# Fabstir/fabstir-vectordb

Hardware: NVIDIA B200
Metric: QPS @ recall@10>=0.95, 1M x 384 IVF (higher is better)
Workload: dtype f32

## Files before the change

### fabstir_vectordb_b200/csrc/common.cuh

```cuda
#pragma once

#include <cuda_runtime.h>
#include <stdint.h>

#include <string>

namespace fvdb {

constexpr uint64_t KEY_NONE = 0xFFFFFFFFFFFFFFFFull;
constexpr uint32_t ID_NONE = 0xFFFFFFFFu;

__host__ __device__ __forceinline__ uint64_t make_key(float dist, uint32_t id) {
#ifdef __CUDA_ARCH__
    return ((uint64_t)__float_as_uint(dist) << 32) | id;
#else
    union { float f; uint32_t u; } c;
    c.f = dist;
    return ((uint64_t)c.u << 32) | id;
#endif
}
__host__ __device__ __forceinline__ uint32_t key_id(uint64_t k) { return (uint32_t)k; }
__device__ __forceinline__ float key_dist(uint64_t k) { return __uint_as_float((uint32_t)(k >> 32)); }

constexpr int METRIC_L2 = 0, METRIC_COS = 1, METRIC_DOT = 2;
// ... 92 lines not shown
        for (int j = 0; j < 8; ++j) {
            const float4 qq = q4[i + j];
            float t, u;
            t = __fsub_rn(qq.x, x[j].x); u = __fsub_rn(qq.x, y[j].x);
            acc0 = __fadd_rn(acc0, __fmul_rn(t, t)); acc1 = __fadd_rn(acc1, __fmul_rn(u, u));
            t = __fsub_rn(qq.y, x[j].y); u = __fsub_rn(qq.y, y[j].y);
            acc0 = __fadd_rn(acc0, __fmul_rn(t, t)); acc1 = __fadd_rn(acc1, __fmul_rn(u, u));
            t = __fsub_rn(qq.z, x[j].z); u = __fsub_rn(qq.z, y[j].z);
            acc0 = __fadd_rn(acc0, __fmul_rn(t, t)); acc1 = __fadd_rn(acc1, __fmul_rn(u, u));
            t = __fsub_rn(qq.w, x[j].w); u = __fsub_rn(qq.w, y[j].w);
            acc0 = __fadd_rn(acc0, __fmul_rn(t, t)); acc1 = __fadd_rn(acc1, __fmul_rn(u, u));
        }
    }
    for (; i < n4; ++i) {
        const float4 xx = __ldg(a4 + i), yy = __ldg(b4 + i), qq = q4[i];
        float t, u;
        t = __fsub_rn(qq.x, xx.x); u = __fsub_rn(qq.x, yy.x);
        acc0 = __fadd_rn(acc0, __fmul_rn(t, t)); acc1 = __fadd_rn(acc1, __fmul_rn(u, u));
        t = __fsub_rn(qq.y, xx.y); u = __fsub_rn(qq.y, yy.y);
        acc0 = __fadd_rn(acc0, __fmul_rn(t, t)); acc1 = __fadd_rn(acc1, __fmul_rn(u, u));
        t = __fsub_rn(qq.z, xx.z); u = __fsub_rn(qq.z, yy.z);
        acc0 = __fadd_rn(acc0, __fmul_rn(t, t)); acc1 = __fadd_rn(acc1, __fmul_rn(u, u));
        t = __fsub_rn(qq.w, xx.w); u = __fsub_rn(qq.w, yy.w);
        acc0 = __fadd_rn(acc0, __fmul_rn(t, t)); acc1 = __fadd_rn(acc1, __fmul_rn(u, u));
    }
    d0 = __fsqrt_rn(acc0);
    d1 = __fsqrt_rn(acc1);
}
#endif

inline int div_up(int a, int b) { return (a + b - 1) / b; }
inline uint64_t div_up64(uint64_t a, uint64_t b) { return (a + b - 1) / b; }

}
```

### fabstir_vectordb_b200/csrc/exact_scan.cu

```cuda
#include "common.cuh"
#include "kernels.cuh"

namespace fvdb {

namespace {

constexpr int TQ = 32;
constexpr int TR = 128;
constexpr int DK = 32;
constexpr int NT = 256;
constexpr int QS_LD = TQ + 4;
constexpr int XS_LD = TR + 4;

__device__ __forceinline__ void warp_insert(uint64_t* list, int k, uint64_t cand, int lane) {
    int cnt = 0;
    for (int i = lane; i < k; i += 32) cnt += (list[i] <= cand) ? 1 : 0;
#pragma unroll
    for (int o = 16; o > 0; o >>= 1) cnt += __shfl_xor_sync(0xffffffffu, cnt, o);
    const int pos = cnt;
    for (int base = ((k - 1) / 32) * 32; base >= 0 && base + 31 > pos; base -= 32) {
        int i = base + lane;
        uint64_t tmp = 0;
        bool mv = (i > pos) && (i < k);
        if (mv) tmp = list[i - 1];
// ... 233 lines not shown
    const uint32_t qt = i / nsplit, sp = i % nsplit;
    const uint32_t rows = row_end - row_begin;
    const uint32_t tiles = (rows + TR - 1) / TR;
    const uint32_t t0 = (uint32_t)(((uint64_t)tiles * sp) / nsplit);
    const uint32_t t1 = (uint32_t)(((uint64_t)tiles * (sp + 1)) / nsplit);
    ScanItem it;
    it.row_begin = row_begin + t0 * TR;
    it.row_end = min(row_end, row_begin + t1 * TR);
    it.pair_begin = qt * TQ;
    it.pair_count = min((uint32_t)TQ, nq - qt * TQ);
    it.slot = sp;
    it.identity = 1;
    it.sub = 0;
    if (it.row_begin >= it.row_end) it.pair_count = 0;
    items[i] = it;
}

cudaError_t launch_build_identity_items(ScanItem* items, uint32_t nq, uint32_t row_begin,
                                        uint32_t row_end, uint32_t nsplit, uint32_t* n_items_out,
                                        cudaStream_t stream) {
    const uint32_t n_qt = (nq + TQ - 1) / TQ;
    const uint32_t n = n_qt * nsplit;
    *n_items_out = n;
    if (n == 0) return cudaSuccess;
    build_identity_items_kernel<<<(n + 255) / 256, 256, 0, stream>>>(items, nq, row_begin, row_end,
                                                                    nsplit);
    return cudaGetLastError();
}

uint32_t exact_scan_tq() { return TQ; }
uint32_t exact_scan_tr() { return TR; }


constexpr uint32_t NEAREST_BIT = 0x80000000u;
__global__ void probe_hist_kernel(const uint64_t* __restrict__ coarse_keys, uint32_t n_pairs,
                                  uint32_t nprobe, uint32_t* __restrict__ list_cnt) {
    const uint32_t i = blockIdx.x * blockDim.x + threadIdx.x;
    if (i >= n_pairs) return;
    const uint64_t key = coarse_keys[i];
    if (key == KEY_NONE) return;
    atomicAdd(&list_cnt[key_id(key)], 1u);
    if (i % nprobe == 0) atomicOr(&list_cnt[key_id(key)], NEAREST_BIT);
}

__device__ __forceinline__ uint64_t block_excl_scan_u64(uint64_t v, uint64_t* warp_tot, uint64_t* total) {
    const int lane = threadIdx.x & 31, w = threadIdx.x >> 5;
    uint64_t inc = v;
#pragma unroll
    for (int o = 1; o < 32; o <<= 1) {
        const uint64_t n = __shfl_up_sync(0xffffffffu, inc, o);
        if (lane >= o) inc += n;
    }
    if (lane == 31) warp_tot[w] = inc;
    __syncthreads();
    if (w == 0) {
        uint64_t t = warp_tot[lane];
        uint64_t ti = t;
#pragma unroll
        for (int o = 1; o < 32; o <<= 1) {
            const uint64_t n = __shfl_up_sync(0xffffffffu, ti, o);
            if (lane >= o) ti += n;
        }
        warp_tot[lane] = ti - t;
        if (lane == 31) warp_tot[32] = ti;
    }
    __syncthreads();
    const uint64_t r = warp_tot[w] + inc - v;
// ... 106 lines not shown
        if (t == 0) *(wide ? n_items_w : n_items) = (uint32_t)(carry >> 32);
        pair_carry = carry & 0xFFFFFFFFull;
    }
    uint64_t rows_total;
    block_excl_scan_u64(my_rows, warp_tot, &rows_total);
    if (t == 0) {
        pair_off[nlist] = (uint32_t)pair_carry;
        if (scanned_rows) *scanned_rows = rows_total;
    }
}

__global__ void probe_scatter_kernel(const uint64_t* __restrict__ coarse_keys, uint32_t n_pairs,
                                     uint32_t nprobe, const uint32_t* __restrict__ list_off,
                                     uint32_t* __restrict__ cursor, uint32_t* __restrict__ pair_q,
                                     uint32_t* __restrict__ pair_slot) {
    const uint32_t i = blockIdx.x * blockDim.x + threadIdx.x;
    if (i >= n_pairs) return;
    const uint64_t key = coarse_keys[i];
    if (key == KEY_NONE) return;
    const uint32_t l = key_id(key);
    if (list_off[l + 1] == list_off[l]) return;
    const uint32_t p = atomicAdd(&cursor[l], 1u);
    pair_q[p] = i / nprobe;
    pair_slot[p] = i % nprobe;
}

cudaError_t launch_probe_bucketing(const uint64_t* coarse_keys, uint32_t nq, uint32_t nprobe,
                                   const uint32_t* list_off, uint32_t nlist, uint32_t tile_q,
                                   uint32_t* list_cnt, uint32_t* pair_off, uint32_t* cursor,
                                   uint32_t* pair_q, uint32_t* pair_slot, ScanItem* items,
                                   uint32_t* n_items, uint64_t* scanned_rows, cudaStream_t stream,
                                   const uint32_t* list_order, bool order_near, uint32_t rows_cap,
                                   uint32_t wide_min, uint32_t tile_q_w, ScanItem* items_w, uint32_t* n_items_w,
                                   bool wide_longest_first, const uint32_t* live_ids, uint32_t n_live) {
    const uint32_t n_pairs = nq * nprobe;
    cudaError_t e = cudaMemsetAsync(list_cnt, 0, sizeof(uint32_t) * nlist, stream);
    if (e != cudaSuccess) return e;
    if (n_pairs == 0) {
        if (wide_min) { e = cudaMemsetAsync(n_items_w, 0, sizeof(uint32_t), stream); if (e != cudaSuccess) return e; }
        return cudaMemsetAsync(n_items, 0, sizeof(uint32_t), stream);
    }
    probe_hist_kernel<<<(n_pairs + 255) / 256, 256, 0, stream>>>(coarse_keys, n_pairs, nprobe, list_cnt);
    probe_scan_kernel<<<1, 1024, 0, stream>>>(list_cnt, list_off, list_order, nlist, tile_q, pair_off, cursor,
                                              items, n_items, scanned_rows, order_near, rows_cap, wide_min, tile_q_w,
                                              items_w, n_items_w, wide_longest_first, live_ids, n_live);
    probe_scatter_kernel<<<(n_pairs + 255) / 256, 256, 0, stream>>>(coarse_keys, n_pairs, nprobe,
                                                                   list_off, cursor, pair_q,
                                                                   pair_slot);
    return cudaGetLastError();
}

__global__ void __launch_bounds__(128) exact_pair_scan_kernel(const uint64_t* __restrict__ coarse_keys, uint32_t n_pairs,
                                                              const uint32_t* __restrict__ list_off,
                                                              const float* __restrict__ X, const uint32_t* __restrict__ ids,
                                                              const float* __restrict__ Q, uint32_t D, uint32_t nprobe,
                                                              uint32_t P, uint32_t k, const uint64_t* __restrict__ tomb,
                                                              uint64_t tomb_bits, const uint64_t* __restrict__ filt,
                                                              uint64_t filt_bits, uint64_t* __restrict__ partial) {
    extern __shared__ __align__(16) unsigned char pair_smem[];
    const int lane = threadIdx.x & 31, w = threadIdx.x >> 5;
    const uint32_t pair = blockIdx.x;
    float* q_s = reinterpret_cast<float*>(pair_smem);
    uint64_t* list = reinterpret_cast<uint64_t*>(pair_smem + (((size_t)D * sizeof(float) + 15) & ~(size_t)15)) + (size_t)w * k;
    const uint32_t q = pair / nprobe, slot = pair % nprobe;
    const uint64_t ck = coarse_keys[pair];
    if (ck == KEY_NONE) return;
    const uint32_t l = key_id(ck);
    const uint32_t b = list_off[l], e = list_off[l + 1];
    for (uint32_t d = threadIdx.x; d < D; d += 128) q_s[d] = __ldg(Q + (size_t)q * D + d);
    for (uint32_t i = lane; i < k; i += 32) list[i] = KEY_NONE;
    __syncthreads();
    uint64_t thr = KEY_NONE;
    for (uint32_t r0 = b + w * 32; r0 < e; r0 += 128) {
        const uint32_t r = r0 + lane;
        uint64_t key = KEY_NONE;
// ... 304 lines not shown
```

### fabstir_vectordb_b200/csrc/kernels.cuh

```cuda
#pragma once

#include "common.cuh"

namespace fvdb {

struct ExactScanArgs {
    const float* X;
    const uint32_t* ids;
    const float* Q;
    uint32_t D;
    const ScanItem* items;
    const uint32_t* item_count;
    uint32_t n_items;
    const uint32_t* pair_q;
    const uint32_t* pair_slot;
    uint32_t P;
    uint32_t k;
    const uint64_t* tomb;
    uint64_t tomb_bits;
    const uint64_t* filt;
    uint64_t filt_bits;
    uint64_t* partial;
    int metric = 0;
};

size_t exact_scan_smem_bytes(uint32_t k);
uint32_t exact_scan_tq();
uint32_t exact_scan_tr();
cudaError_t launch_exact_scan(const ExactScanArgs& a, uint32_t grid, cudaStream_t stream);
cudaError_t launch_build_identity_items(ScanItem* items, uint32_t nq, uint32_t row_begin,
                                        uint32_t row_end, uint32_t nsplit, uint32_t* n_items_out,
                                        cudaStream_t stream);
cudaError_t launch_probe_bucketing(const uint64_t* coarse_keys, uint32_t nq, uint32_t nprobe,
                                   const uint32_t* list_off, uint32_t nlist, uint32_t tile_q,
                                   uint32_t* list_cnt, uint32_t* pair_off, uint32_t* cursor,
                                   uint32_t* pair_q, uint32_t* pair_slot, ScanItem* items,
                                   uint32_t* n_items, uint64_t* scanned_rows, cudaStream_t stream,
                                   const uint32_t* list_order = nullptr, bool order_near = false,
                                   uint32_t rows_cap = 0,
                                   uint32_t wide_min = 0, uint32_t tile_q_w = 0, ScanItem* items_w = nullptr,
                                   uint32_t* n_items_w = nullptr, bool wide_longest_first = false,
                                   const uint32_t* live_ids = nullptr, uint32_t n_live = 0);
cudaError_t launch_exact_pair_scan(const uint64_t* coarse_keys, uint32_t nq, uint32_t nprobe, const uint32_t* list_off,
                                   const float* X, const uint32_t* ids, const float* Q, uint32_t D, uint32_t P,
                                   uint32_t k, const uint64_t* tomb, uint64_t tomb_bits, const uint64_t* filt,
                                   uint64_t filt_bits, uint64_t* partial, cudaStream_t stream);
cudaError_t launch_merge_partials(const uint64_t* in, uint32_t nq, uint32_t P, uint32_t k,
                                  uint64_t* out, cudaStream_t stream);
cudaError_t launch_merge_rows32(const uint64_t* in, uint32_t nq, uint32_t P, uint64_t* out,
                                cudaStream_t stream, const uint32_t* row_stamp, uint32_t stamp);
cudaError_t launch_finalize(const uint64_t* recent, const uint64_t* ivf, uint32_t nq, uint32_t k,
                            uint32_t* out_ids, float* out_dist, uint32_t* out_count,
                            cudaStream_t stream, int metric = 0, uint32_t* ivf_ids = nullptr,
                            float* ivf_dist = nullptr, uint32_t* ivf_count = nullptr);
cudaError_t launch_merge_parts(const uint32_t* ids, const float* dist, const uint32_t* cnt,
                               uint32_t parts, uint32_t nq, uint32_t k, uint32_t* out_ids,
                               float* out_dist, uint32_t* out_count, cudaStream_t stream,
                               size_t stride_kv = 0, size_t stride_c = 0, bool tiered = false);
cudaError_t launch_scatter_result_rows(const uint32_t* ids, const float* dist, const uint32_t* cnt,
                                       const uint32_t* idx, uint32_t n, uint32_t k, uint32_t* out_ids,
                                       float* out_dist, uint32_t* out_cnt, cudaStream_t stream);
cudaError_t launch_postfilter_rows(const uint32_t* ids, const float* dist, const uint32_t* cnt, uint32_t nq,
                                   uint32_t k3, uint32_t k, const uint64_t* keep, uint64_t keep_bits,
                                   uint32_t* out_ids, float* out_dist, uint32_t* out_cnt, cudaStream_t stream);
cudaError_t launch_scatter_keys(const uint64_t* src, const uint32_t* idx, uint32_t n, uint32_t k,
                                uint64_t* dst, cudaStream_t stream);
cudaError_t launch_nan_check(const float* x, size_t n, int* flag, cudaStream_t stream);

size_t stable_group_scratch_bytes(uint64_t n, uint32_t nkeys);
cudaError_t launch_stable_group(const uint32_t* keys, uint64_t n, uint32_t nkeys, uint32_t* offsets,
                                uint32_t* perm, void* scratch, cudaStream_t stream);
cudaError_t launch_gather_rows(const float* src0, uint64_t n0, const float* src1, const uint32_t* perm,
                               uint64_t n, uint32_t D, float* dst, cudaStream_t stream);
cudaError_t launch_gather_u32(const uint32_t* src0, uint64_t n0, const uint32_t* src1,
                              const uint32_t* perm, uint64_t n, uint32_t* dst, cudaStream_t stream);
// ... 28 lines not shown
```

### fabstir_vectordb_b200/csrc/tc_scan.cu

```cuda
#include <cuda.h>
#include <cuda_runtime.h>

#include <algorithm>
#include <cmath>
#include <cstdio>
#include <cstdlib>
#include <vector>

#include "../../include/fvdb.h"
#include "kernels.cuh"
#include "tc_ptx.cuh"
#include "tc_scan.cuh"

namespace fvdb {

namespace {

constexpr int TC_ROWS = 128;
constexpr int TC_KB_FLOATS = 32;
constexpr int TC_KP = 32;
constexpr int TC_THREADS = 192;

struct TcScanParams {
    const ScanItem* items;
// ... 969 lines not shown
                buf ^= 1;
            }
            Q1_LAP(6);
        }
        if (warp == 2) Q1_LAP_DUMP(2);
    }
    tc_fence_before();
    __syncthreads();
    if (warp == 1) {
        tc_fence_after();
        asm volatile("tcgen05.dealloc.cta_group::1.sync.aligned.b32 %0, %1;" ::"r"(tmem_base),
                     "r"((uint32_t)Q1_TMEM_COLS)
                     : "memory");
    }
}

size_t tc_scan_q_smem_bytes(uint32_t stages, uint32_t kbs) {
    return (size_t)stages * kbs * Q1_STAGE_BYTES + (size_t)2 * Q1_M * Q1_XP_LD * 4 + (size_t)Q1_NSLOT * Q1_N * 4 +
           (size_t)(2 * stages + 5 + 2 * TC_SCHED + Q1_NSLOT) * 8 + 16 + (size_t)TC_SCHED * 4;
}

uint32_t q1_pick_stages(uint32_t KB, uint32_t kbs) {
    const uint32_t nst = KB / kbs;
    uint32_t stages = std::min<uint32_t>(18u, (uint32_t)(Q1_NSLOT - 4) * nst);
    while (stages > 2 && tc_scan_q_smem_bytes(stages, kbs) + 1024 > 232448) --stages;
    return stages;
}


#include "tc_scan_wide.cuh"

__global__ void row_norms_kernel(const float* __restrict__ x, uint64_t n, uint32_t D, float* __restrict__ out,
                                 uint32_t* __restrict__ max_bits, uint32_t* __restrict__ fill = nullptr,
                                 uint32_t fill_value = 0, int* __restrict__ nan_flag = nullptr) {
    const uint64_t w = ((uint64_t)blockIdx.x * blockDim.x + threadIdx.x) >> 5;
    const int lane = threadIdx.x & 31;
    const uint64_t nw = ((uint64_t)gridDim.x * blockDim.x) >> 5;
    float mx = 0.f;
    for (uint64_t r = w; r < n; r += nw) {
        const float4* row = reinterpret_cast<const float4*>(x + (size_t)r * D);
        float s = 0.f;
        for (uint32_t c = lane; c < D / 4; c += 32) {
            const float4 v = __ldg(row + c);
            s = fmaf(v.x, v.x, s); s = fmaf(v.y, v.y, s); s = fmaf(v.z, v.z, s); s = fmaf(v.w, v.w, s);
        }
#pragma unroll
        for (int o = 16; o > 0; o >>= 1) s += __shfl_xor_sync(0xffffffffu, s, o);
        if (lane == 0) {
            out[r] = s;
            if (fill) fill[r] = fill_value;
            if (nan_flag && isnan(s)) *nan_flag = 1;
        }
        mx = fmaxf(mx, s);
    }
    if (max_bits && lane == 0 && mx > 0.f) atomicMax(max_bits, __float_as_uint(mx));
}

__global__ void fill_u32_kernel(uint32_t* __restrict__ p, uint64_t n, uint32_t v) {
    uint64_t i = (uint64_t)blockIdx.x * blockDim.x + threadIdx.x;
    const uint64_t stride = (uint64_t)gridDim.x * blockDim.x;
    for (; i < n; i += stride) p[i] = v;
}

constexpr int GATHER_STAGES_ROWS = 6;
constexpr int GATHER_STAGES_CENT = 4;
__host__ __device__ constexpr int gather_warp_bytes(int stages) { return stages * 32 * 128; }
template <int GATHER_STAGES, int METRIC = METRIC_L2>
// ... 158 lines not shown
    it.slot = it.row_begin;
    it.identity = 1;
    it.sub = 0;
    if (it.row_begin >= it.row_end) it.pair_count = 0;
    items[i] = it;
}

__global__ void flat_items_kernel(ScanItem* items, uint32_t nq, uint32_t n_rows, uint32_t chunk_rows,
                                  uint32_t n_chunks, uint32_t* n_items, uint32_t tile_q) {
    const uint32_t n_qg = (nq + tile_q - 1) / tile_q;
    const uint32_t i = blockIdx.x * blockDim.x + threadIdx.x;
    if (i == 0) *n_items = n_qg * n_chunks;
    if (i >= n_qg * n_chunks) return;
    const uint32_t c = i / n_qg, g = i % n_qg;
    ScanItem it;
    it.row_begin = c * chunk_rows;
    it.row_end = min(n_rows, (c + 1) * chunk_rows);
    it.pair_begin = g * tile_q;
    it.pair_count = min(tile_q, nq - g * tile_q);
    it.slot = c;
    it.identity = n_qg > 1 ? 2 : 1;
    it.sub = 0;
    if (it.row_begin >= it.row_end) it.pair_count = 0;
    items[i] = it;
}

template <int T>
__global__ void __launch_bounds__(128) coarse_select_kernel(const float* __restrict__ dense, uint32_t ld,
                                                            const float* __restrict__ centroids,
                                                            const float* __restrict__ Q, const float* __restrict__ qnorm,
                                                            const uint32_t* __restrict__ cmax_bits, uint32_t nq,
                                                            uint32_t nlist, uint32_t D, uint32_t np, uint32_t KC,
                                                            uint64_t* __restrict__ out_keys,
                                                            uint32_t* __restrict__ fb_count, uint32_t* __restrict__ fb_idx) {
    constexpr int GWB = gather_warp_bytes(GATHER_STAGES_CENT);
    extern __shared__ __align__(128) unsigned char cs_sm[];
    const int tid = threadIdx.x, lane = tid & 31, w = tid >> 5;
    const uint32_t q = blockIdx.x;
    const uint32_t nw = (KC + 31) / 32;
    float* q_s = reinterpret_cast<float*>(cs_sm + (size_t)nw * GWB);
    uint32_t* cand_s = reinterpret_cast<uint32_t*>(q_s + D);
    uint32_t* red_s = cand_s + 128;
    uint64_t* key_s = reinterpret_cast<uint64_t*>(red_s + 32);
    for (uint32_t d = tid; d < D; d += 128) q_s[d] = __ldg(Q + (size_t)q * D + d);
    uint32_t ld2[T], lid[T];
#pragma unroll
    for (int i = 0; i < T; ++i) { ld2[i] = 0xFFFFFFFFu; lid[i] = 0xFFFFFFFFu; }
    const float* row = dense + (size_t)q * ld;
    for (uint32_t base = 0; base < nlist; base += 1024) {
        float v[8];
#pragma unroll
        for (int i = 0; i < 8; ++i) {
            const uint32_t c = base + (uint32_t)i * 128u + (uint32_t)tid;
            v[i] = (c < nlist) ? __ldg(row + c) : 0.0f;
        }
#pragma unroll
        for (int i2 = 0; i2 < 8; ++i2) {
            const uint32_t c = base + (uint32_t)i2 * 128u + (uint32_t)tid;
            uint32_t kd = __float_as_uint(fmaxf(v[i2], 0.0f)), ki = c;
            if (c < nlist && kd < ld2[T - 1]) {
#pragma unroll
                for (int i = 0; i < T; ++i) {
                    const bool sw = kd < ld2[i];
                    const uint32_t td = sw ? ld2[i] : kd, ti = sw ? lid[i] : ki;
                    ld2[i] = sw ? kd : ld2[i];
                    lid[i] = sw ? ki : lid[i];
                    kd = td; ki = ti;
// ... 98 lines not shown
        }
        key_s[tid] = key;
    }
    __syncthreads();
    if (w != 0) return;
    uint64_t ex[4];
#pragma unroll
    for (int ch = 0; ch < 4; ++ch) {
        ex[ch] = KEY_NONE;
        if ((uint32_t)ch * 32 < KC) ex[ch] = warp_sort32(key_s[ch * 32 + lane], lane);
    }
#pragma unroll
    for (int a2 = 0; a2 < 3; ++a2) {
#pragma unroll
        for (int b2 = 3; b2 > a2; --b2) {
            if ((uint32_t)b2 * 32 >= KC) continue;
            const uint64_t rev = shfl64(ex[b2], 31 - lane);
            uint64_t lo = ex[b2 - 1] < rev ? ex[b2 - 1] : rev;
            uint64_t hi = ex[b2 - 1] < rev ? rev : ex[b2 - 1];
#pragma unroll
            for (int j = 16; j > 0; j >>= 1) {
                const uint64_t ol = shfl_xor64(lo, j), oh = shfl_xor64(hi, j);
                const bool lower = (lane & j) == 0;
                lo = lower ? (lo < ol ? lo : ol) : (lo < ol ? ol : lo);
                hi = lower ? (hi < oh ? hi : oh) : (hi < oh ? oh : hi);
            }
            ex[b2 - 1] = lo;
            ex[b2] = hi;
        }
    }
#pragma unroll
    for (int i = 0; i < 4; ++i) {
        const uint32_t o = i * 32 + lane;
        if (o < np) out_keys[(size_t)q * np + o] = ex[i];
    }
    uint64_t kth = KEY_NONE;
#pragma unroll
    for (int i = 0; i < 4; ++i) if ((int)((np - 1) >> 5) == i) kth = shfl64(ex[i], (int)((np - 1) & 31));
    if (lane == 0) {
        bool ok = true;
        if (uncertain) ok = false;
        else if (next_d2 != 0xFFFFFFFFu) {
            const float a_next = __uint_as_float(next_d2);
            const float cmax = sqrtf(__uint_as_float(*cmax_bits));
            const float eps = 1.05f * 0.00390625f * sqrtf(qnorm[q]) * cmax + 3.1e-5f * a_next + 1e-30f;
            ok = false;
            if (kth != KEY_NONE) {
                const float dk = key_dist(kth);
                ok = (a_next - eps) > dk * dk * 1.000001f;
            }
        }
#ifdef FVDB_CS_DEBUG
        if (!ok) printf("coarse_select q %u uncertain %d next_d2 %08x (%f) kth %f KCe %u t %08x\n", q, (int)uncertain, next_d2,
                        __uint_as_float(next_d2), kth != KEY_NONE ? key_dist(kth) * key_dist(kth) : -1.f, KCe, t);
#endif
        if (!ok) fb_idx[atomicAdd(fb_count, 1u)] = q;
    }
}

__global__ void __launch_bounds__(128) merge_rows32_kernel(const uint64_t* __restrict__ in, uint32_t nq, uint32_t P,
                                                           uint64_t* __restrict__ out,
                                                           const uint32_t* __restrict__ row_stamp, uint32_t stamp) {
    __shared__ uint64_t part[3][32];
    const int lane = threadIdx.x & 31, w = threadIdx.x >> 5;
    const uint32_t q = blockIdx.x;
    const uint64_t* base = in + (size_t)q * P * TC_KP;
    const uint32_t* st_q = row_stamp + (size_t)q * P;
// ... 129 lines not shown
    return cudaGetLastError();
}

cudaError_t launch_fill_u32(uint32_t* p, uint64_t n, uint32_t v, cudaStream_t stream) {
    if (n == 0) return cudaSuccess;
    fill_u32_kernel<<<(uint32_t)((n + 255) / 256), 256, 0, stream>>>(p, n, v);
    return cudaGetLastError();
}

cudaError_t launch_merge_rows32(const uint64_t* in, uint32_t nq, uint32_t P, uint64_t* out, cudaStream_t stream,
                                const uint32_t* row_stamp, uint32_t stamp) {
    if (nq == 0) return cudaSuccess;
    merge_rows32_kernel<<<nq, 128, 0, stream>>>(in, nq, P, out, row_stamp, stamp);
    return cudaGetLastError();
}

struct TcScratchImpl {
    Buf<float> xnorm, qnorm;
    Buf<uint32_t> misc;
    Buf<unsigned long long> prof;
    Buf<uint32_t> list_order;
    Buf<uint32_t> live_ids;
    uint32_t n_live = 0;
    struct RowSet {
        Buf<float> xnorm;
        CUtensorMap tmap;
        CUtensorMap tmap_w;
        const float* rows = nullptr;
        uint64_t n = 0, version = ~0ull;
    } rs[2];
    Buf<ScanItem> fitems;
    uint32_t list_order_n = 0;
    uint32_t max_list_len = 0;
    Buf<uint32_t> thr_g, list_cnt, pair_off, cursor, pair_q, pair_slot, n_items;
    Buf<ScanItem> items, items_w;
    Buf<uint64_t> partial, shortlist;
    Buf<uint32_t> row_stamp;
    uint32_t stamp = 0;
    cudaError_t next_stamp(size_t rows, size_t* dev_bytes, cudaStream_t st, uint32_t* out) {
        const size_t before = row_stamp.cap;
        cudaError_t e = row_stamp.ensure(rows, dev_bytes);
        if (e != cudaSuccess) return e;
        if (row_stamp.cap != before || stamp == 0xFFFFFFFFu) {
            e = cudaMemsetAsync(row_stamp.p, 0, row_stamp.cap * sizeof(uint32_t), st);
            if (e != cudaSuccess) return e;
            stamp = 0;
        }
        *out = ++stamp;
        return cudaSuccess;
    }
    Buf<float> cnorm, dense;
    Buf<uint64_t> coarse;
    Buf<ScanItem> citems;
    CUtensorMap tmap_cent;
    const float* tmap_cent_ptr = nullptr;
    uint32_t tmap_cent_n = 0;
    CUtensorMap tmap_arena;
    CUtensorMap tmap_w;
    uint32_t smem_attr_set_w = 0;
    bool smem_attr_set_q = false;
    const float* tmap_rows = nullptr;
    uint64_t tmap_n = 0;
    bool smem_attr_set = false;
    bool smem_attr_set_rerank = false;
    cudaStream_t side = nullptr;
    cudaEvent_t ev_fork = nullptr, ev_join = nullptr;
};

bool tc_supported(uint32_t D) { return D % 32 == 0 && D >= 32 && D <= 512; }

static size_t rerank_smem_bytes(uint32_t D) { return (size_t)4 * gather_warp_bytes(GATHER_STAGES_ROWS) + (size_t)4 * D * sizeof(float); }
static size_t coarse_select_smem_bytes(uint32_t D, uint32_t KC) {
    return (size_t)((KC + 31) / 32) * gather_warp_bytes(GATHER_STAGES_CENT) + (size_t)D * sizeof(float) + (128 + 32) * 4 + 128 * 8;
}
static cudaError_t rerank_prepare(TcScratchImpl* m) {
    if (m->smem_attr_set_rerank) return cudaSuccess;
    cudaError_t e = cudaFuncSetAttribute(rerank_kernel<METRIC_L2>, cudaFuncAttributeMaxDynamicSharedMemorySize, (int)rerank_smem_bytes(512));
    if (e == cudaSuccess) e = cudaFuncSetAttribute(rerank_kernel<METRIC_COS>, cudaFuncAttributeMaxDynamicSharedMemorySize, (int)rerank_smem_bytes(512));
    if (e == cudaSuccess) e = cudaFuncSetAttribute(rerank_kernel<METRIC_DOT>, cudaFuncAttributeMaxDynamicSharedMemorySize, (int)rerank_smem_bytes(512));
    if (e == cudaSuccess) e = cudaFuncSetAttribute(coarse_select_kernel<8>, cudaFuncAttributeMaxDynamicSharedMemorySize, (int)coarse_select_smem_bytes(512, 128));
    if (e == cudaSuccess) m->smem_attr_set_rerank = true;
    return e;
}

void tc_release(TcScratch& s) {
    if (!s.impl) return;
    TcScratchImpl* m = s.impl;
    m->xnorm.release(); m->qnorm.release(); m->misc.release(); m->thr_g.release(); m->list_cnt.release();
    m->pair_off.release(); m->cursor.release(); m->pair_q.release(); m->pair_slot.release(); m->n_items.release();
    m->items.release(); m->items_w.release(); m->partial.release(); m->shortlist.release(); m->row_stamp.release();
    m->prof.release(); m->list_order.release(); m->live_ids.release(); m->rs[0].xnorm.release(); m->rs[1].xnorm.release(); m->fitems.release();
    m->cnorm.release(); m->dense.release(); m->coarse.release(); m->citems.release();
    if (m->ev_fork) cudaEventDestroy(m->ev_fork);
    if (m->ev_join) cudaEventDestroy(m->ev_join);
    if (m->side) cudaStreamDestroy(m->side);
    delete m;
    s.impl = nullptr;
}

#define TCK(call)                                                                      \
    do {                                                                               \
        cudaError_t e__ = (call);                                                      \
        if (e__ != cudaSuccess) {                                                      \
            if (err) *err = std::string("CUDA error: ") + cudaGetErrorString(e__) + " at " #call; \
            cudaGetLastError();                                                        \
            return e__ == cudaErrorMemoryAllocation ? FVDB_ERR_OOM : FVDB_ERR_CUDA;    \
        }                                                                              \
    } while (0)

static char tc_kernel_choice(uint32_t D, int sm_count) {
    const char* kenv = getenv("FVDB_TC_KERNEL");
    char c = (kenv && kenv[0] == 'R') ? 'R' : 'W';
    if (c == 'W' && (D > 384 || sm_count < 2)) c = 'R';
    return c;
}

static cudaError_t launch_wide(TcScratchImpl* m, const CUtensorMap& tmap, TcScanParams& p, uint32_t KB, int sm_count,
                               size_t* dev_bytes, cudaStream_t st, cudaEvent_t ev0) {
    const uint32_t kbs = wide_pick_kbs(KB);
    uint32_t stages = wide_pick_stages(KB, kbs);
    if (const char* e = getenv("FVDB_TC_STAGES")) { const uint32_t v = (uint32_t)atoi(e); if (v >= 2 && v < stages) stages = v; }
// ... 103 lines not shown
            TCK(cudaStreamSynchronize(st));
            m->list_order_n = a.nlist;
        }
        m->tmap_rows = a.rows;
        m->tmap_n = a.n_rows;
        s.arena_dirty = false;
    }

    const size_t n_pairs = (size_t)nq * np;
    const char kch = tc_kernel_choice(D, a.sm_count);
    uint32_t wide_min = 0;
    if (kch == 'W') {
        wide_min = TC_WIDE_MIN_QUERIES;
        if (const char* e = getenv("FVDB_TC_WIDE_MIN")) wide_min = (uint32_t)std::max(1, atoi(e));
    }
    const bool use_wide = wide_min != 0;
    const uint32_t tile_q = TC_TILE_Q;
    uint32_t n_split = 1, rows_cap = 0;
    {
        uint32_t want = TC_SPLIT_MAX;
        if (const char* e = getenv("FVDB_TC_SPLIT")) want = std::min<uint32_t>(std::max(1, atoi(e)), 16u);
        const uint32_t unit = (uint32_t)R2_ROWS;
        if (want > 1 && m->max_list_len > TC_SPLIT_MIN_ROWS) {
            rows_cap = std::max<uint32_t>(TC_SPLIT_MIN_ROWS / 2, ((m->max_list_len + want - 1) / want + unit - 1) / unit * unit);
            n_split = (m->max_list_len + rows_cap - 1) / rows_cap;
            if (n_split <= 1) { n_split = 1; rows_cap = 0; }
        }
    }
    const uint32_t prows = (use_wide ? (uint32_t)W_SUBROWS : 1u) * n_split;
    const size_t max_items = ((size_t)a.nlist + (n_pairs + tile_q - 1) / tile_q) * n_split + 1;
    const size_t max_items_w = use_wide ? ((size_t)a.nlist + (n_pairs + W_NQ - 1) / W_NQ) * n_split + 1 : 0;
    TCK(m->qnorm.ensure(nq, dev_bytes));
    TCK(m->thr_g.ensure(nq, dev_bytes));
    TCK(m->list_cnt.ensure(a.nlist + 1, dev_bytes));
    TCK(m->pair_off.ensure(a.nlist + 2, dev_bytes));
    TCK(m->cursor.ensure(a.nlist + 1, dev_bytes));
    TCK(m->pair_q.ensure(n_pairs, dev_bytes));
    TCK(m->pair_slot.ensure(n_pairs, dev_bytes));
    TCK(m->n_items.ensure(8, dev_bytes));
    TCK(m->items.ensure(max_items, dev_bytes));
    if (use_wide) TCK(m->items_w.ensure(max_items_w, dev_bytes));
    TCK(m->partial.ensure(n_pairs * prows * TC_KP, dev_bytes));
    TCK(m->shortlist.ensure((size_t)nq * TC_KP, dev_bytes));

    {
        const uint32_t blocks = (uint32_t)std::min<uint64_t>(((uint64_t)nq * 32 + 255) / 256, (uint64_t)a.sm_count * 8);
        const char* dbg = getenv("FVDB_TC_DEBUG");
        const bool reset_bounds = !(dbg && (atoi(dbg) & 512)) && !a.thr_ext;
        row_norms_kernel<<<blocks, 256, 0, st>>>(a.Q, nq, D, m->qnorm.p, nullptr, reset_bounds ? m->thr_g.p : nullptr,
                                                 F32_INF_BITS, a.d_nan);
        TCK(cudaGetLastError());
        (*launches) += 1;
    }
    const uint64_t* coarse_keys = a.coarse_keys;
    if (!coarse_keys) {
        if (D > 384 || np > TC_MAX_NPROBE_COARSE) { if (err) *err = "TC coarse step unsupported for this shape"; return FVDB_ERR_INVALID_ARG; }
        if (s.centroids_dirty || m->tmap_cent_ptr != a.centroids || m->tmap_cent_n != a.nlist) {
            TCK(m->cnorm.ensure(a.nlist, dev_bytes));
            TCK(cudaMemsetAsync(m->misc.p + 4, 0, 4, st));
            const uint32_t blocks = (uint32_t)std::min<uint64_t>(((uint64_t)a.nlist * 32 + 255) / 256, (uint64_t)a.sm_count * 8);
            row_norms_kernel<<<blocks, 256, 0, st>>>(a.centroids, a.nlist, D, m->cnorm.p, m->misc.p + 4);
            TCK(cudaGetLastError());
            (*launches)++;
            EncodeTiledFn enc = get_encode_fn();
            if (!enc) { if (err) *err = "cuTensorMapEncodeTiled unavailable"; return FVDB_ERR_CUDA; }
            const cuuint64_t gdim[2] = {D, a.nlist};
            const cuuint64_t gstride[1] = {(cuuint64_t)D * 4};
            const cuuint32_t box[2] = {TC_KB_FLOATS, Q1_N};
            const cuuint32_t estr[2] = {1, 1};
            CUresult r = enc(&m->tmap_cent, CU_TENSOR_MAP_DATA_TYPE_FLOAT32, 2, const_cast<float*>(a.centroids), gdim,
                             gstride, box, estr, CU_TENSOR_MAP_INTERLEAVE_NONE, CU_TENSOR_MAP_SWIZZLE_128B,
                             CU_TENSOR_MAP_L2_PROMOTION_L2_256B, CU_TENSOR_MAP_FLOAT_OOB_FILL_NONE);
            if (r != CUDA_SUCCESS) { if (err) *err = "cuTensorMapEncodeTiled (centroids) failed"; return FVDB_ERR_CUDA; }
            m->tmap_cent_ptr = a.centroids;
            m->tmap_cent_n = a.nlist;
            s.centroids_dirty = false;
        }
        const uint32_t ld = (a.nlist + 63) / 64 * 64;
        const uint32_t n_qg = (nq + Q1_M - 1) / Q1_M;
        const uint32_t tiles = ld / 64;
        uint32_t n_chunks = std::max(1u, std::min(tiles, ((uint32_t)a.sm_count + n_qg - 1) / n_qg));
        const uint32_t chunk_rows = ((tiles + n_chunks - 1) / n_chunks) * 64;
        n_chunks = (ld + chunk_rows - 1) / chunk_rows;
        const uint32_t n_citems = n_qg * n_chunks;
        TCK(m->dense.ensure((size_t)nq * ld, dev_bytes));
        TCK(m->coarse.ensure((size_t)nq * np, dev_bytes));
        TCK(m->citems.ensure(n_citems, dev_bytes));
        coarse_items_kernel<<<(n_citems + 127) / 128, 128, 0, st>>>(m->citems.p, nq, a.nlist, chunk_rows, n_chunks,
                                                                     m->n_items.p + 2);
        TCK(cudaGetLastError());
        TcScanParams cp{};
        cp.items = m->citems.p; cp.item_count = m->n_items.p + 2; cp.Q = a.Q; cp.qnorm = m->qnorm.p; cp.D = D; cp.KB = KB;
        cp.xnorm = m->cnorm.p; cp.ids = nullptr; cp.P = 1; cp.partial = nullptr; cp.thr_g = nullptr;
        cp.work_counter = m->n_items.p + 3;
        TCK(cudaMemsetAsync(cp.work_counter, 0, 4, st));
        cp.dense_out = m->dense.p; cp.dense_ld = ld;
        uint32_t kbs = 1;
        for (uint32_t c : {4u, 3u, 2u}) if (KB % c == 0) { kbs = c; break; }
        uint32_t stages = q1_pick_stages(KB, kbs);
        cp.stages = stages; cp.kbs = kbs;
        if (!m->smem_attr_set_q) {
            TCK(cudaFuncSetAttribute(tc_scan_q_kernel, cudaFuncAttributeMaxDynamicSharedMemorySize, 232448));
            m->smem_attr_set_q = true;
        }
        tc_scan_q_kernel<<<std::min<uint32_t>((uint32_t)a.sm_count, n_citems), TC_THREADS,
                           tc_scan_q_smem_bytes(stages, kbs) + 1024, st>>>(m->tmap_cent, cp);
        TCK(cudaGetLastError());
        const uint32_t KC = std::min(np + 32, 128u);
        const size_t sel_smem = coarse_select_smem_bytes(D, KC);
        TCK(rerank_prepare(m));
        coarse_select_kernel<8><<<nq, 128, sel_smem, st>>>(m->dense.p, ld, a.centroids, a.Q, m->qnorm.p,
                                                          m->misc.p + 4, nq, a.nlist, D, np, KC,
                                                          m->coarse.p, a.d_fallback_count, a.d_fallback_idx);
        TCK(cudaGetLastError());
        (*launches) += 3;
        coarse_keys = m->coarse.p;
        if (a.coarse_out) TCK(cudaMemcpyAsync(a.coarse_out, m->coarse.p, (size_t)nq * np * 8, cudaMemcpyDeviceToDevice, st));
    }
    if (a.coarse_only) return FVDB_OK;
    TCK(launch_probe_bucketing(coarse_keys, nq, np, a.list_off, a.nlist, tile_q, m->list_cnt.p, m->pair_off.p,
                               m->cursor.p, m->pair_q.p, m->pair_slot.p, m->items.p, m->n_items.p, a.d_scanned_rows, st,
                               (m->list_order_n == a.nlist && !getenv("FVDB_TC_NO_ORDER")) ? m->list_order.p : nullptr,
                               getenv("FVDB_TC_ORDER_NEAR") != nullptr, rows_cap, wide_min, (uint32_t)W_NQ,
                               use_wide ? m->items_w.p : nullptr, m->n_items.p + 6, getenv("FVDB_TC_W_ORDER") != nullptr,
                               (m->list_order_n == a.nlist && !getenv("FVDB_TC_NO_ORDER")) ? m->live_ids.p : nullptr, m->n_live));
    (*launches) += 3;
    uint32_t stamp = 0;
    TCK(m->next_stamp(n_pairs * prows, dev_bytes, st, &stamp));

    TcScanParams p{};
    p.items = m->items.p; p.item_count = m->n_items.p; p.pair_q = m->pair_q.p; p.pair_slot = m->pair_slot.p;
    p.Q = a.Q; p.qnorm = m->qnorm.p; p.D = D; p.KB = KB; p.xnorm = m->xnorm.p; p.ids = a.ids;
    p.tomb = a.tomb; p.tomb_bits = a.tomb_bits; p.filt = a.filt; p.filt_bits = a.filt_bits;
    p.P = np; p.S = prows; p.partial = m->partial.p; p.thr_g = a.thr_ext ? a.thr_ext : m->thr_g.p;
    p.row_stamp = m->row_stamp.p; p.stamp = stamp;
    p.n_peer = a.thr_ext ? std::min(a.n_peers, TC_MAX_PEERS) : 0u;
    for (uint32_t r = 0; r < p.n_peer; ++r) p.thr_peer[r] = a.thr_peers[r];
    p.rows_raw = a.rows; p.rows_bytes = a.n_rows * (uint64_t)D * 4;
    p.work_counter = m->n_items.p + 1;
    {
        const char* dbg = getenv("FVDB_TC_DEBUG");
        p.debug = dbg ? (uint32_t)atoi(dbg) : 0u;
    }
    const bool wide_first_env = [] { const char* oe = getenv("FVDB_TC_ORDER"); return oe && oe[0] == 'W'; }();
    const bool fork_wide = use_wide && !wide_first_env && !(p.debug & 128u) && getenv("FVDB_TC_FORK") != nullptr;
    if (fork_wide && !m->side) {
        TCK(cudaStreamCreateWithFlags(&m->side, cudaStreamNonBlocking));
        TCK(cudaEventCreateWithFlags(&m->ev_fork, cudaEventDisableTiming));
        TCK(cudaEventCreateWithFlags(&m->ev_join, cudaEventDisableTiming));
    }
    p.scan_sms = a.scan_sms;
    TCK(cudaMemsetAsync(p.work_counter, 0, 4, st));
    if (use_wide) TCK(cudaMemsetAsync(m->n_items.p + 7, 0, 4, st));
    if (a.wait_before_scan) TCK(cudaStreamWaitEvent(st, a.wait_before_scan, 0));
    if (a.ev_scan0) TCK(cudaEventRecord(a.ev_scan0, st));
    if (fork_wide) TCK(cudaEventRecord(m->ev_fork, st));
    auto run_wide = [&]() -> int {
    if (use_wide) {
        TcScanParams pw = p;
        pw.items = m->items_w.p; pw.item_count = m->n_items.p + 6; pw.work_counter = m->n_items.p + 7;
        if (fork_wide) {
            TCK(cudaStreamWaitEvent(m->side, m->ev_fork, 0));
            TCK(launch_wide(m, m->tmap_w, pw, KB, a.sm_count, dev_bytes, m->side, nullptr));
            TCK(cudaEventRecord(m->ev_join, m->side));
            TCK(cudaStreamWaitEvent(st, m->ev_join, 0));
        } else {
            TCK(launch_wide(m, m->tmap_w, pw, KB, a.sm_count, dev_bytes, st, nullptr));
        }
        (*launches)++;
    }
    return FVDB_OK;
    };
    auto run_narrow = [&]() -> int {
    {
        uint32_t stages = std::min<uint32_t>(12u, (uint32_t)(R2_NSLOT - 2 - R2_NBUF) * KB);
        while (stages > 2 && tc_scan_smem_bytes(KB, stages) + R2_SLACK > 232448) --stages;
        if (const char* e = getenv("FVDB_TC_STAGES")) { const uint32_t v = (uint32_t)atoi(e); if (v >= 2 && v < stages) stages = v; }
        p.stages = stages;
        const size_t smem = tc_scan_smem_bytes(KB, stages) + R2_SLACK;
        if (smem > 232448) { if (err) *err = "TC scan does not fit shared memory for this dim"; return FVDB_ERR_INVALID_CONFIG; }
        if (!m->smem_attr_set) {
            TCK(cudaFuncSetAttribute(tc_scan_kernel, cudaFuncAttributeMaxDynamicSharedMemorySize, 232448));
            m->smem_attr_set = true;
        }
        uint32_t grid = (uint32_t)std::min<size_t>((size_t)a.sm_count, max_items);
        if (p.scan_sms && p.scan_sms < grid) grid = p.scan_sms;
        if (p.debug & 128u) {
            TCK(m->prof.ensure((size_t)grid * 48, dev_bytes));
            TCK(cudaMemsetAsync(m->prof.p, 0, (size_t)grid * 48 * 8, st));
            p.prof = m->prof.p;
        }
        tc_scan_kernel<<<grid, R2_THREADS, smem, st>>>(m->tmap_arena, p);
        TCK(cudaGetLastError());
// ... 133 lines not shown
```

Baseline: 2.189 million.

## Fuse per-batch zeroing and probe histogram into existing kernels, cache coarse items

```diff
diff --git a/fabstir_vectordb_b200/csrc/common.cuh b/fabstir_vectordb_b200/csrc/common.cuh
--- a/fabstir_vectordb_b200/csrc/common.cuh
+++ b/fabstir_vectordb_b200/csrc/common.cuh
@@ -148,4 +148,6 @@
 inline int div_up(int a, int b) { return (a + b - 1) / b; }
 inline uint64_t div_up64(uint64_t a, uint64_t b) { return (a + b - 1) / b; }
 
+constexpr uint32_t NEAREST_BIT = 0x80000000u;
+
 }
diff --git a/fabstir_vectordb_b200/csrc/exact_scan.cu b/fabstir_vectordb_b200/csrc/exact_scan.cu
--- a/fabstir_vectordb_b200/csrc/exact_scan.cu
+++ b/fabstir_vectordb_b200/csrc/exact_scan.cu
@@ -289,7 +289,6 @@
 uint32_t exact_scan_tr() { return TR; }
 
 
-constexpr uint32_t NEAREST_BIT = 0x80000000u;
 __global__ void probe_hist_kernel(const uint64_t* __restrict__ coarse_keys, uint32_t n_pairs,
                                   uint32_t nprobe, uint32_t* __restrict__ list_cnt) {
     const uint32_t i = blockIdx.x * blockDim.x + threadIdx.x;
@@ -462,15 +461,18 @@
                                    uint32_t* n_items, uint64_t* scanned_rows, cudaStream_t stream,
                                    const uint32_t* list_order, bool order_near, uint32_t rows_cap,
                                    uint32_t wide_min, uint32_t tile_q_w, ScanItem* items_w, uint32_t* n_items_w,
-                                   bool wide_longest_first, const uint32_t* live_ids, uint32_t n_live) {
+                                   bool wide_longest_first, const uint32_t* live_ids, uint32_t n_live, bool hist_done) {
     const uint32_t n_pairs = nq * nprobe;
-    cudaError_t e = cudaMemsetAsync(list_cnt, 0, sizeof(uint32_t) * nlist, stream);
-    if (e != cudaSuccess) return e;
+    cudaError_t e = cudaSuccess;
     if (n_pairs == 0) {
         if (wide_min) { e = cudaMemsetAsync(n_items_w, 0, sizeof(uint32_t), stream); if (e != cudaSuccess) return e; }
         return cudaMemsetAsync(n_items, 0, sizeof(uint32_t), stream);
     }
-    probe_hist_kernel<<<(n_pairs + 255) / 256, 256, 0, stream>>>(coarse_keys, n_pairs, nprobe, list_cnt);
+    if (!hist_done) {
+        e = cudaMemsetAsync(list_cnt, 0, sizeof(uint32_t) * nlist, stream);
+        if (e != cudaSuccess) return e;
+        probe_hist_kernel<<<(n_pairs + 255) / 256, 256, 0, stream>>>(coarse_keys, n_pairs, nprobe, list_cnt);
+    }
     probe_scan_kernel<<<1, 1024, 0, stream>>>(list_cnt, list_off, list_order, nlist, tile_q, pair_off, cursor,
                                               items, n_items, scanned_rows, order_near, rows_cap, wide_min, tile_q_w,
                                               items_w, n_items_w, wide_longest_first, live_ids, n_live);
diff --git a/fabstir_vectordb_b200/csrc/kernels.cuh b/fabstir_vectordb_b200/csrc/kernels.cuh
--- a/fabstir_vectordb_b200/csrc/kernels.cuh
+++ b/fabstir_vectordb_b200/csrc/kernels.cuh
@@ -40,7 +40,8 @@
                                    uint32_t rows_cap = 0,
                                    uint32_t wide_min = 0, uint32_t tile_q_w = 0, ScanItem* items_w = nullptr,
                                    uint32_t* n_items_w = nullptr, bool wide_longest_first = false,
-                                   const uint32_t* live_ids = nullptr, uint32_t n_live = 0);
+                                   const uint32_t* live_ids = nullptr, uint32_t n_live = 0,
+                                   bool hist_done = false);
 cudaError_t launch_exact_pair_scan(const uint64_t* coarse_keys, uint32_t nq, uint32_t nprobe, const uint32_t* list_off,
                                    const float* X, const uint32_t* ids, const float* Q, uint32_t D, uint32_t P,
                                    uint32_t k, const uint64_t* tomb, uint64_t tomb_bits, const uint64_t* filt,
diff --git a/fabstir_vectordb_b200/csrc/tc_scan.cu b/fabstir_vectordb_b200/csrc/tc_scan.cu
--- a/fabstir_vectordb_b200/csrc/tc_scan.cu
+++ b/fabstir_vectordb_b200/csrc/tc_scan.cu
@@ -1025,7 +1025,9 @@
 
 __global__ void row_norms_kernel(const float* __restrict__ x, uint64_t n, uint32_t D, float* __restrict__ out,
                                  uint32_t* __restrict__ max_bits, uint32_t* __restrict__ fill = nullptr,
-                                 uint32_t fill_value = 0, int* __restrict__ nan_flag = nullptr) {
+                                 uint32_t fill_value = 0, int* __restrict__ nan_flag = nullptr,
+                                 uint32_t* __restrict__ zero = nullptr, uint32_t n_zero = 0) {
+    for (uint32_t i = blockIdx.x * blockDim.x + threadIdx.x; i < n_zero; i += gridDim.x * blockDim.x) zero[i] = 0;
     const uint64_t w = ((uint64_t)blockIdx.x * blockDim.x + threadIdx.x) >> 5;
     const int lane = threadIdx.x & 31;
     const uint64_t nw = ((uint64_t)gridDim.x * blockDim.x) >> 5;
@@ -1250,7 +1252,8 @@
                                                             const uint32_t* __restrict__ cmax_bits, uint32_t nq,
                                                             uint32_t nlist, uint32_t D, uint32_t np, uint32_t KC,
                                                             uint64_t* __restrict__ out_keys,
-                                                            uint32_t* __restrict__ fb_count, uint32_t* __restrict__ fb_idx) {
+                                                            uint32_t* __restrict__ fb_count, uint32_t* __restrict__ fb_idx,
+                                                            uint32_t* __restrict__ list_cnt) {
     constexpr int GWB = gather_warp_bytes(GATHER_STAGES_CENT);
     extern __shared__ __align__(128) unsigned char cs_sm[];
     const int tid = threadIdx.x, lane = tid & 31, w = tid >> 5;
@@ -1415,7 +1418,13 @@
 #pragma unroll
     for (int i = 0; i < 4; ++i) {
         const uint32_t o = i * 32 + lane;
-        if (o < np) out_keys[(size_t)q * np + o] = ex[i];
+        if (o < np) {
+            out_keys[(size_t)q * np + o] = ex[i];
+            if (ex[i] != KEY_NONE) {
+                atomicAdd(&list_cnt[key_id(ex[i])], 1u);
+                if (o == 0) atomicOr(&list_cnt[key_id(ex[i])], NEAREST_BIT);
+            }
+        }
     }
     uint64_t kth = KEY_NONE;
 #pragma unroll
@@ -1611,7 +1620,9 @@
     Buf<ScanItem> fitems;
     uint32_t list_order_n = 0;
     uint32_t max_list_len = 0;
-    Buf<uint32_t> thr_g, list_cnt, pair_off, cursor, pair_q, pair_slot, n_items;
+    Buf<uint32_t> thr_g, pair_off, cursor, pair_q, pair_slot, n_items;
+    Buf<uint32_t> batch_zero;
+    static constexpr uint32_t BZ_R = 0, BZ_W = 1, BZ_COARSE = 2, BZ_LIST_CNT = 3;
     Buf<ScanItem> items, items_w;
     Buf<uint64_t> partial, shortlist;
     Buf<uint32_t> row_stamp;
@@ -1631,6 +1642,7 @@
     Buf<float> cnorm, dense;
     Buf<uint64_t> coarse;
     Buf<ScanItem> citems;
+    uint32_t citems_nq = 0, citems_nlist = 0, citems_sms = 0;
     CUtensorMap tmap_cent;
     const float* tmap_cent_ptr = nullptr;
     uint32_t tmap_cent_n = 0;
@@ -1665,7 +1677,7 @@
 void tc_release(TcScratch& s) {
     if (!s.impl) return;
     TcScratchImpl* m = s.impl;
-    m->xnorm.release(); m->qnorm.release(); m->misc.release(); m->thr_g.release(); m->list_cnt.release();
+    m->xnorm.release(); m->qnorm.release(); m->misc.release(); m->thr_g.release(); m->batch_zero.release();
     m->pair_off.release(); m->cursor.release(); m->pair_q.release(); m->pair_slot.release(); m->n_items.release();
     m->items.release(); m->items_w.release(); m->partial.release(); m->shortlist.release(); m->row_stamp.release();
     m->prof.release(); m->list_order.release(); m->live_ids.release(); m->rs[0].xnorm.release(); m->rs[1].xnorm.release(); m->fitems.release();
@@ -1835,7 +1847,8 @@
     const size_t max_items_w = use_wide ? ((size_t)a.nlist + (n_pairs + W_NQ - 1) / W_NQ) * n_split + 1 : 0;
     TCK(m->qnorm.ensure(nq, dev_bytes));
     TCK(m->thr_g.ensure(nq, dev_bytes));
-    TCK(m->list_cnt.ensure(a.nlist + 1, dev_bytes));
+    TCK(m->batch_zero.ensure(TcScratchImpl::BZ_LIST_CNT + a.nlist + 1, dev_bytes));
+    uint32_t* const list_cnt = m->batch_zero.p + TcScratchImpl::BZ_LIST_CNT;
     TCK(m->pair_off.ensure(a.nlist + 2, dev_bytes));
     TCK(m->cursor.ensure(a.nlist + 1, dev_bytes));
     TCK(m->pair_q.ensure(n_pairs, dev_bytes));
@@ -1851,7 +1864,8 @@
         const char* dbg = getenv("FVDB_TC_DEBUG");
         const bool reset_bounds = !(dbg && (atoi(dbg) & 512)) && !a.thr_ext;
         row_norms_kernel<<<blocks, 256, 0, st>>>(a.Q, nq, D, m->qnorm.p, nullptr, reset_bounds ? m->thr_g.p : nullptr,
-                                                 F32_INF_BITS, a.d_nan);
+                                                 F32_INF_BITS, a.d_nan, m->batch_zero.p,
+                                                 TcScratchImpl::BZ_LIST_CNT + a.nlist + 1);
         TCK(cudaGetLastError());
         (*launches) += 1;
     }
@@ -1888,15 +1902,18 @@
         const uint32_t n_citems = n_qg * n_chunks;
         TCK(m->dense.ensure((size_t)nq * ld, dev_bytes));
         TCK(m->coarse.ensure((size_t)nq * np, dev_bytes));
-        TCK(m->citems.ensure(n_citems, dev_bytes));
-        coarse_items_kernel<<<(n_citems + 127) / 128, 128, 0, st>>>(m->citems.p, nq, a.nlist, chunk_rows, n_chunks,
-                                                                     m->n_items.p + 2);
-        TCK(cudaGetLastError());
+        if (m->citems_nq != nq || m->citems_nlist != a.nlist || m->citems_sms != (uint32_t)a.sm_count) {
+            TCK(m->citems.ensure(n_citems, dev_bytes));
+            coarse_items_kernel<<<(n_citems + 127) / 128, 128, 0, st>>>(m->citems.p, nq, a.nlist, chunk_rows, n_chunks,
+                                                                         m->n_items.p + 2);
+            TCK(cudaGetLastError());
+            (*launches)++;
+            m->citems_nq = nq; m->citems_nlist = a.nlist; m->citems_sms = (uint32_t)a.sm_count;
+        }
         TcScanParams cp{};
         cp.items = m->citems.p; cp.item_count = m->n_items.p + 2; cp.Q = a.Q; cp.qnorm = m->qnorm.p; cp.D = D; cp.KB = KB;
         cp.xnorm = m->cnorm.p; cp.ids = nullptr; cp.P = 1; cp.partial = nullptr; cp.thr_g = nullptr;
-        cp.work_counter = m->n_items.p + 3;
-        TCK(cudaMemsetAsync(cp.work_counter, 0, 4, st));
+        cp.work_counter = m->batch_zero.p + TcScratchImpl::BZ_COARSE;
         cp.dense_out = m->dense.p; cp.dense_ld = ld;
         uint32_t kbs = 1;
         for (uint32_t c : {4u, 3u, 2u}) if (KB % c == 0) { kbs = c; break; }
@@ -1914,20 +1931,22 @@
         TCK(rerank_prepare(m));
         coarse_select_kernel<8><<<nq, 128, sel_smem, st>>>(m->dense.p, ld, a.centroids, a.Q, m->qnorm.p,
                                                           m->misc.p + 4, nq, a.nlist, D, np, KC,
-                                                          m->coarse.p, a.d_fallback_count, a.d_fallback_idx);
+                                                          m->coarse.p, a.d_fallback_count, a.d_fallback_idx, list_cnt);
         TCK(cudaGetLastError());
-        (*launches) += 3;
+        (*launches) += 2;
         coarse_keys = m->coarse.p;
         if (a.coarse_out) TCK(cudaMemcpyAsync(a.coarse_out, m->coarse.p, (size_t)nq * np * 8, cudaMemcpyDeviceToDevice, st));
     }
     if (a.coarse_only) return FVDB_OK;
-    TCK(launch_probe_bucketing(coarse_keys, nq, np, a.list_off, a.nlist, tile_q, m->list_cnt.p, m->pair_off.p,
+    const bool hist_done = !a.coarse_keys;
+    TCK(launch_probe_bucketing(coarse_keys, nq, np, a.list_off, a.nlist, tile_q, list_cnt, m->pair_off.p,
                                m->cursor.p, m->pair_q.p, m->pair_slot.p, m->items.p, m->n_items.p, a.d_scanned_rows, st,
                                (m->list_order_n == a.nlist && !getenv("FVDB_TC_NO_ORDER")) ? m->list_order.p : nullptr,
                                getenv("FVDB_TC_ORDER_NEAR") != nullptr, rows_cap, wide_min, (uint32_t)W_NQ,
                                use_wide ? m->items_w.p : nullptr, m->n_items.p + 6, getenv("FVDB_TC_W_ORDER") != nullptr,
-                               (m->list_order_n == a.nlist && !getenv("FVDB_TC_NO_ORDER")) ? m->live_ids.p : nullptr, m->n_live));
-    (*launches) += 3;
+                               (m->list_order_n == a.nlist && !getenv("FVDB_TC_NO_ORDER")) ? m->live_ids.p : nullptr, m->n_live,
+                               hist_done));
+    (*launches) += hist_done ? 2 : 3;
     uint32_t stamp = 0;
     TCK(m->next_stamp(n_pairs * prows, dev_bytes, st, &stamp));
 
@@ -1940,7 +1959,7 @@
     p.n_peer = a.thr_ext ? std::min(a.n_peers, TC_MAX_PEERS) : 0u;
     for (uint32_t r = 0; r < p.n_peer; ++r) p.thr_peer[r] = a.thr_peers[r];
     p.rows_raw = a.rows; p.rows_bytes = a.n_rows * (uint64_t)D * 4;
-    p.work_counter = m->n_items.p + 1;
+    p.work_counter = m->batch_zero.p + TcScratchImpl::BZ_R;
     {
         const char* dbg = getenv("FVDB_TC_DEBUG");
         p.debug = dbg ? (uint32_t)atoi(dbg) : 0u;
@@ -1953,15 +1972,13 @@
         TCK(cudaEventCreateWithFlags(&m->ev_join, cudaEventDisableTiming));
     }
     p.scan_sms = a.scan_sms;
-    TCK(cudaMemsetAsync(p.work_counter, 0, 4, st));
-    if (use_wide) TCK(cudaMemsetAsync(m->n_items.p + 7, 0, 4, st));
     if (a.wait_before_scan) TCK(cudaStreamWaitEvent(st, a.wait_before_scan, 0));
     if (a.ev_scan0) TCK(cudaEventRecord(a.ev_scan0, st));
     if (fork_wide) TCK(cudaEventRecord(m->ev_fork, st));
     auto run_wide = [&]() -> int {
     if (use_wide) {
         TcScanParams pw = p;
-        pw.items = m->items_w.p; pw.item_count = m->n_items.p + 6; pw.work_counter = m->n_items.p + 7;
+        pw.items = m->items_w.p; pw.item_count = m->n_items.p + 6; pw.work_counter = m->batch_zero.p + TcScratchImpl::BZ_W;
         if (fork_wide) {
             TCK(cudaStreamWaitEvent(m->side, m->ev_fork, 0));
             TCK(launch_wide(m, m->tmap_w, pw, KB, a.sm_count, dev_bytes, m->side, nullptr));
```

New measurement: 2.236 million, median of 6. +2.1%, better.
